# hruffieux/atlasqtl

Hardware: AMD Instinct MI355X
Metric: VB sweeps/sec (higher is better)
Workload: dtype f64; 1 GPU; atlasqtl VB sweep (S1-S22 incl. scheduled ELBO), n=1000 p=50000 q=10000, anneal=(1,2,10) on, horseshoe global-local, sweeps 6-93; n=1000, p=50000, q=10000, q_per_gpu=10000, parallelism=trait-sharded x1, env_overrides=

## Files before the change

atlasqtl_amd/csrc/aq_core_sweep_la.h:

```cpp
#pragma once
#include <hip/hip_runtime.h>
#include "aq_core_sweep.h"
#include <type_traits>

typedef double aq_v2 __attribute__((ext_vector_type(2)));

__device__ __forceinline__ double aq_row16_sum(double v) {
  auto step = [&](auto ctrl) __attribute__((always_inline)) {
    constexpr int C = decltype(ctrl)::value;
    const int lo = __builtin_amdgcn_update_dpp(0, __double2loint(v), C, 0xf, 0xf, false);
    const int hi = __builtin_amdgcn_update_dpp(0, __double2hiint(v), C, 0xf, 0xf, false);
    v += __hiloint2double(hi, lo);
  };
  step(std::integral_constant<int, 0xB1>{});
  step(std::integral_constant<int, 0x4E>{});
  step(std::integral_constant<int, 0x124>{});
  step(std::integral_constant<int, 0x128>{});
  return v;
}

#ifndef AQ_GLDS_AUX
#define AQ_GLDS_AUX 2
#endif
__device__ __forceinline__ void aq_glds16(const void *gsrc_lane, void *lds_base) {
  __builtin_amdgcn_global_load_lds((const __attribute__((address_space(1))) void *)gsrc_lane,
                                   (__attribute__((address_space(3))) void *)lds_base, 16, 0, AQ_GLDS_AUX);
}

template <int... Is, class F>
__device__ __forceinline__ void aq_static_for_impl(std::integer_sequence<int, Is...>, F &&f) {
  (f(std::integral_constant<int, Is>{}), ...);
}
template <int N, class F>
__device__ __forceinline__ void aq_static_for(F &&f) {
  aq_static_for_impl(std::make_integer_sequence<int, N>{}, f);
}

#define AQ_LD2(d0, d1, voff, sbase)                                                                            \
  do {                                                                                                          \
    const unsigned long long b_ = (unsigned long long)(sbase);                                                  \
    const unsigned lo_ = __builtin_amdgcn_readfirstlane((unsigned)b_);                                          \
    const unsigned hi_ = __builtin_amdgcn_readfirstlane((unsigned)(b_ >> 32));                                  \
    const unsigned long long u_ = ((unsigned long long)hi_ << 32) | lo_;                                        \
    asm volatile("global_load_dwordx4 %0, %2, %3\n\tglobal_load_dwordx4 %1, %2, %3 offset:1024"                \
                 : "=&v"(d0), "=&v"(d1)                                                                         \
                 : "v"(voff), "s"(u_));                                                                         \
  } while (0)
#define AQ_LD2I(d0, d1, voff, sbase, IMM)                                                                      \
  do {                                                                                                          \
    const unsigned long long b_ = (unsigned long long)(sbase);                                                  \
    const unsigned lo_ = __builtin_amdgcn_readfirstlane((unsigned)b_);                                          \
    const unsigned hi_ = __builtin_amdgcn_readfirstlane((unsigned)(b_ >> 32));                                  \
    const unsigned long long u_ = ((unsigned long long)hi_ << 32) | lo_;                                        \
    asm volatile("global_load_dwordx4 %0, %2, %3 offset:%4\n\tglobal_load_dwordx4 %1, %2, %3 offset:%5"        \
                 : "=&v"(d0), "=&v"(d1)                                                                         \
                 : "v"(voff), "s"(u_), "i"(IMM), "i"((IMM) + 1024));                                            \
  } while (0)
#define AQ_WAIT2(N, d0, d1) asm volatile("s_waitcnt vmcnt(" #N ")" : "+v"(d0), "+v"(d1))
template <int N>
__device__ __forceinline__ void aq_wait2n(aq_v2 &d0, aq_v2 &d1) {
  static_assert(N >= 0 && N < 64, "vmcnt is a 6-bit field");
  asm volatile("s_waitcnt vmcnt(%2)" : "+v"(d0), "+v"(d1) : "n"(N));
}

constexpr int aq_req_index(int D, int last, int stream , int k) {
  int n = 0;
  for (int j = 0; j <= D - 2; j++) {
    if (stream == 0 && k == j) return n;
    n++;
    if (j <= D - 3) {
      if (stream == 1 && k == j) return n;
      n++;
    }
  }
  for (int t = 0; t <= last; t++) {
    if (t + D - 1 <= last) {
      if (stream == 0 && k == t + D - 1) return n;
      n++;
    }
    if (t + D - 2 <= last) {
      if (stream == 1 && k == t + D - 2) return n;
      n++;
    }
  }
  return -1;
}
constexpr int aq_req_issued(int D, int last, int t) {
  int n = (D - 1) + (D - 2);
  for (int s = 0; s <= t; s++) n += (s + D - 1 <= last) + (s + D - 2 <= last);
  return n;
}
#ifndef AQ_DEEP_TT1
#define AQ_DEEP_TT1 4
#endif

template <int NT, int NT2, bool SEG, int TT, bool MASK = false, int NT3_ = -1, bool WIDE = false>
__global__ __launch_bounds__(8 * 64, 2) void aq_core_sweep_la_kernel(const AqCoreArgs a) {
  static_assert(!MASK || TT == 1, "the masked form keeps 16 per-trait Gram blocks in LDS: one trait tile per workgroup");
  static_assert(!WIDE || (TT == 1 && !SEG), "the wide sample split: one trait tile per workgroup, never chained");
  constexpr int NWM = 6;
  constexpr int NT3 = NT3_ >= 0 ? NT3_ : aq_la_nt3(NT, NT2, TT);
  constexpr int NPS = NWM + (NT3 > 0 ? 1 : 0);
  constexpr int NTR = 16 * TT;
  constexpr int ENT = 256 * TT;
  constexpr int NG = 4 / TT;
  constexpr int RPG = 16 / NG;
  const int tid = threadIdx.x;
  const int lane = tid & 63;
  const int w = tid >> 6;
  const bool is_rec = (w == 3);
  const int mw = w < 3 ? w : w - 1;
  const int g = lane >> 4;
  const int col = lane & 15;
  const int nwg = a.ntile / TT;
  int wg_ = blockIdx.x, seg_b0 = 0, seg_b1 = a.nb, seg = 0;
  if (SEG) {
    seg = blockIdx.x / nwg;
    wg_ = blockIdx.x - seg * nwg;
    seg_b0 = (int)((long long)a.nb * seg / a.nseg);
    seg_b1 = (int)((long long)a.nb * (seg + 1) / a.nseg);
    if (seg > 0) {
      if (tid == 0) {
        int tries = 0;
        while (__hip_atomic_load(&a.done[wg_], __ATOMIC_RELAXED, __HIP_MEMORY_SCOPE_AGENT) < seg) {
          __builtin_amdgcn_s_sleep(32);
          if (++tries > 4000000) { *a.errflag = 1; break; }
        }
        __builtin_amdgcn_fence(__ATOMIC_ACQUIRE, "agent");
        asm volatile("s_waitcnt vmcnt(0)" ::: "memory");
      }
      __syncthreads();
    }
  }
  const int C = SEG ? 1 : a.C;
  const int part = C > 1 ? wg_ % C : 0;
  const int wg = C > 1 ? wg_ / C : wg_;
  const bool lead = (part == 0);
  const int tile0 = wg * TT;
  const int nblk = seg_b1 - seg_b0;
  const bool helper = (w == 7);
  const int ht = lane & (NTR - 1), hg = lane / NTR;

  __shared__ double Sp[2][NPS][ENT];
  __shared__ double LA[2][ENT];
  __shared__ double Lm1[2][ENT];
  __shared__ double LB[2][ENT];
  __shared__ double Laa[2][ENT];
  __shared__ double LG[MASK ? 1 : 2][MASK ? 1 : 512];
  constexpr bool CXC = (TT == 1) && !MASK;
  __shared__ double LGx[MASK ? 1 : 3][MASK ? 1 : 256];
  __shared__ double LGk2[MASK ? 2 : 1][MASK ? AQ_GK_DIAG : 1];
  __shared__ double LGxk[MASK ? 4096 : 1];
  __shared__ double Lcoef[2][MASK ? ENT : 1], LK[2][MASK ? ENT : 1], Ls2[2][MASK ? ENT : 1], Lls2[2][MASK ? ENT : 1], Lxn[2][MASK ? ENT : 1];
  __shared__ double Lgam[2][ENT], Lmu[2][ENT], Ldel[2][ENT];
  __shared__ double Lcx[MASK ? 1 : ENT];
  __shared__ double Ldum[ENT];
  __shared__ double Stot[(SEG || TT == 2) ? 1 : 2][(SEG || TT == 2) ? 1 : ENT];
  __shared__ double Lpt[AQ_PT_LEN];
  __shared__ double Lred[6][64];
  __shared__ double Lrn[NPS * 4][NTR];
  __shared__ __attribute__((aligned(16))) int Fl[16];
  typedef __attribute__((address_space(3))) volatile int aq_lds_vint;
  aq_lds_vint *Flv = (aq_lds_vint *)(__attribute__((address_space(3))) int *)Fl;
  auto signal = [&](int idx, int val) __attribute__((always_inline)) {
    asm volatile("s_waitcnt lgkmcnt(0)" ::: "memory");
    if (lane == 0) Flv[idx] = val;
  };
#ifdef AQ_DIAG_TIME
  long long dg_wait = 0, dg_wait_b = 0;
  const long long dg_t0 = __builtin_readcyclecounter();
#endif
#if defined(AQ_DIAG_TIME) || defined(AQ_DIAG_TL)
  auto tl_mark = [&](int i, int k) __attribute__((always_inline)) {
    if (a.dbg && blockIdx.x == 0 && i >= 64 && i < 96 && lane == 0)
      a.dbg[(size_t)gridDim.x * 24 + ((size_t)w * 32 + (i - 64)) * 8 + k] = __builtin_readcyclecounter();
  };
#else
  auto tl_mark = [&](int, int) __attribute__((always_inline)) {};
#endif
  auto wait_ge = [&](int idx, int val) __attribute__((always_inline)) {
#ifdef AQ_DIAG_TIME
    const long long t_in = __builtin_readcyclecounter();
#endif
    while (Flv[idx] < val) __builtin_amdgcn_s_sleep(1);
    asm volatile("" ::: "memory");
#ifdef AQ_DIAG_TIME
    if (idx >= 7) dg_wait_b += __builtin_readcyclecounter() - t_in;
    else dg_wait += __builtin_readcyclecounter() - t_in;
#endif
  };
  typedef int aq_i4 __attribute__((ext_vector_type(4)));
  auto wait_s_and_staged = [&](int val) __attribute__((always_inline)) {
    typedef __attribute__((address_space(3))) volatile aq_i4 aq_lds_vi4;
    aq_lds_vi4 *fp = (aq_lds_vi4 *)(__attribute__((address_space(3))) int *)Fl;
#ifdef AQ_DIAG_TIME
    const long long t_in = __builtin_readcyclecounter();
#endif
    for (;;) {
      const aq_i4 f0 = fp[0], f1 = fp[1];
      const int lo = min(min(min(f0.x, f0.y), min(f0.z, f0.w)), min(min(f1.x, f1.y), f1.w));
      if (lo >= val) break;
      __builtin_amdgcn_s_sleep(1);
    }
    asm volatile("" ::: "memory");
#ifdef AQ_DIAG_TIME
    dg_wait += __builtin_readcyclecounter() - t_in;
#endif
  };
  if (tid < 16) Fl[tid] = 0;

  const int ktrait = tile0 * 16 + ht;
  const bool kvalid = ktrait < a.q;
  double sig2b_k = 1.0;
  if (helper) {
    sig2b_k = a.sig2b[ktrait];
    if (a.mode != 1)
      for (int e = lane; e < AQ_PT_LEN; e += 64) Lpt[e] = aq_pt_dev[e];
#pragma unroll
    for (int r = 0; r < RPG; r++) {
      const int e = lane + 64 * r;
      Ldel[0][e] = Ldel[1][e] = 0.0;
    }
    if constexpr (!MASK) {
#pragma unroll
      for (int r = 0; r < 4; r++) {
        const int e = lane + 64 * r;
        LG[0][(e >> 4) * 32 + 16 + (e & 15)] = 0.0;
        LG[1][(e >> 4) * 32 + 16 + (e & 15)] = 0.0;
      }
    }
  }

  constexpr int NTT = 3 * (NT + NT2) + NT3;
  const int nblk_s = a.mode == 1 ? 0 : nblk;
  auto run = [&](auto ntc, auto rolec, auto hook) __attribute__((always_inline)) {
    constexpr int NTC = decltype(ntc)::value;
    constexpr int ROLE = decltype(rolec)::value;
    constexpr bool HI = ROLE == 0;
    constexpr int ST = (NTC + 2) / 3;
    const int my_t0 = part * NTT + (ROLE == 0 ? mw * NT : ROLE == 1 ? 3 * NT + (mw - 3) * NT2 : 3 * (NT + NT2));
    const int slot = ROLE == 2 ? NWM : mw;
    aq_d4 Rr[TT][NTC];
    unsigned long long mb0 = 0, mb1 = 0;
    aq_static_for<TT>([&](auto ttc) __attribute__((always_inline)) {
      constexpr int tt = decltype(ttc)::value;
      const double *Rg = a.R + (size_t)(tile0 + tt) * a.n_pad * 16 + (size_t)(16 * my_t0 + g) * 16 + col;
      aq_static_for<NTC>([&](auto tc) __attribute__((always_inline)) {
        constexpr int t = decltype(tc)::value;
#pragma unroll
        for (int r = 0; r < 4; r++) Rr[tt][t][r] = Rg[(16 * t + 4 * r) * 16];
        if constexpr (MASK) {
          const double *Mg = a.mis + (size_t)tile0 * a.n_pad * 16 + (size_t)(16 * my_t0 + g) * 16 + col;
#pragma unroll
          for (int r = 0; r < 4; r++)
            if (Mg[(16 * t + 4 * r) * 16] != 0.0) { if (t < 16) mb0 |= 1ull << (4 * (t & 15) + r); else mb1 |= 1ull << (4 * (t & 15) + r); }
        }
      });
    });
    auto remask = [&](auto tc) __attribute__((always_inline)) {
      constexpr int t = decltype(tc)::value;
      const unsigned long long mb = t < 16 ? mb0 : mb1;
#pragma unroll
      for (int r = 0; r < 4; r++) Rr[0][t][r] = ((mb >> (4 * (t & 15) + r)) & 1ull) ? Rr[0][t][r] : 0.0;
    };
    const unsigned voff = (unsigned)((my_t0 * 128 + lane) * 16);
    const char *XUb = (const char *)a.XU, *XAb = (const char *)a.XA;
    const long long BLK = (long long)NTT * C * 128 * 16;
    aq_v2 p0, p1, q0, q1, c0, c1, d0, d1;
#ifdef AQ_FORCE_DEEP_DB
#ifdef AQ_FORCE_DEEP_TT2
    constexpr bool DEEP = (NTC >= 4);
#else
    constexpr bool DEEP = (TT == 1) && (NTC >= 4);
#endif
    constexpr int DB = !DEEP ? 1 : AQ_FORCE_DEEP_DB;
#elif defined(AQ_FORCE_DEEP_MASK_DB)
    constexpr bool DEEP = (TT == 1) && (NTC >= 4) && (MASK || true);
    constexpr int DB = !DEEP ? 1 : MASK ? AQ_FORCE_DEEP_MASK_DB : (NT <= 11) ? AQ_DEEP_TT1 : 3;
#else
    constexpr bool DEEP = (TT == 1) && (NTC >= 4) && (!MASK || (SEG && NT <= 11));
    constexpr int DB = !DEEP ? 1 : (!MASK && NT <= 11) ? AQ_DEEP_TT1 : 3;
#endif
    aq_v2 xb[DB][2], ab[DB][2];
    auto dangling = [&](const char *xu0, const char *xa0, auto skip_first) __attribute__((always_inline)) {
      aq_static_for<DB - 1>([&](auto jc) __attribute__((always_inline)) {
        constexpr int j = decltype(jc)::value;
        if constexpr (!(decltype(skip_first)::value && j == 0)) {
          constexpr int kb = (j + 2) / 4, imm = (j - 4 * kb) * 2048;
          AQ_LD2I(xb[j][0], xb[j][1], voff, xu0 + kb * 8192, imm);
        }
        if constexpr (j <= DB - 3) {
          constexpr int kb = (j + 2) / 4, imm = (j - 4 * kb) * 2048;
          AQ_LD2I(ab[j][0], ab[j][1], voff, xa0 + kb * 8192, imm);
        }
      });
    };
    if constexpr (DEEP) {
      dangling(XUb + seg_b0 * BLK, XAb + seg_b0 * BLK, std::false_type{});
    } else {
      AQ_LD2(p0, p1, voff, XUb + seg_b0 * BLK);
      AQ_LD2(c0, c1, voff, XAb + seg_b0 * BLK);
    }
    for (int i = 0; i <= nblk + 1; i++) {
      const bool do_u = i >= 2, do_s = i < nblk_s;
      const double mflag = do_u ? -1.0 : 0.0;
      const int bu = seg_b0 + (i >= 2 ? i - 2 : 0), bs = seg_b0 + (i < nblk ? i : nblk - 1);
      const int nbu = seg_b0 + (i >= 1 ? (i - 1 < nblk ? i - 1 : nblk - 1) : 0), nbs = seg_b0 + (i + 1 < nblk ? i + 1 : nblk - 1);
      tl_mark(i, 0);
      hook(i);
      tl_mark(i, 1);
      if (do_u && (ROLE != 2 || a.mode == 1)) wait_ge(6, i - 1);
      if (ROLE == 1 && a.stagger) wait_ge(8 + (mw - 3), i + 1);
      tl_mark(i, 2);
      double nd[TT][4];
      {
        unsigned zero = 0;
        asm volatile("" : "+v"(zero));
        const int ln = __builtin_amdgcn_mbcnt_hi(~0u, __builtin_amdgcn_mbcnt_lo(~0u, zero));
        const double *dl = &Ldel[bu & 1][(ln >> 4) * NTR + (ln & 15)];
#pragma unroll
        for (int tt = 0; tt < TT; tt++)
#pragma unroll
// ... 179 lines not shown
      __hip_atomic_store(&slot[(size_t)part * ENT + 64 * r], mine[r], __ATOMIC_RELAXED, __HIP_MEMORY_SCOPE_AGENT);
    }
    meanwhile();
    double tot[RPG];
#pragma unroll
    for (int r = 0; r < RPG; r++) tot[r] = 0.0;
    unsigned long long cur[RPG], nxt[RPG];
    auto request = [&](int c2, unsigned long long (&dst)[RPG]) __attribute__((always_inline)) {
#pragma unroll
      for (int r = 0; r < RPG; r++)
        dst[r] = __hip_atomic_load(&slot[(size_t)c2 * ENT + 64 * r], __ATOMIC_RELAXED, __HIP_MEMORY_SCOPE_AGENT);
    };
    request(part == 0 ? 1 : 0, cur);
    for (int c2 = 0; c2 < C; c2++) {
      if (c2 == part) {
#pragma unroll
        for (int r = 0; r < RPG; r++) tot[r] += __longlong_as_double((long long)mine[r]);
        continue;
      }
      int cn = c2 + 1;
      if (cn == part) cn++;
      if (cn < C) request(cn, nxt);
      int spins = 0;
      for (;;) {
        bool ok = true;
#pragma unroll
        for (int r = 0; r < RPG; r++) ok = ok && ((cur[r] & 3ull) == tag);
        if (__all(ok) || split_dead) break;
        __builtin_amdgcn_s_sleep(1);
        if (++spins > (1 << 22)) { *a.errflag = 1; split_dead = true; }
        request(c2, cur);
      }
#pragma unroll
      for (int r = 0; r < RPG; r++) {
        tot[r] += __longlong_as_double((long long)cur[r]);
        cur[r] = nxt[r];
      }
    }
#pragma unroll
    for (int r = 0; r < RPG; r++) own[r] = tot[r];
  };

  auto split_exchange_wide = [&](int b, double (&own)[RPG], auto meanwhile) __attribute__((always_inline)) {
    static_assert(RPG == 4 && ENT == 256, "one trait tile per workgroup");
    const int par = b & 1;
    const unsigned long long tag = 1ull + (unsigned long long)(((b - seg_b0) >> 1) % 3);
    unsigned long long *slots = (unsigned long long *)a.Pbuf + ((size_t)(wg * 2 + par) * (C + 1)) * ENT;
    tl_mark(b - seg_b0 + 1, 2);
#pragma unroll
    for (int r = 0; r < RPG; r++)
      __hip_atomic_store(&slots[(size_t)part * ENT + lane + 64 * r], ((unsigned long long)__double_as_longlong(own[r]) & ~3ull) | tag,
                         __ATOMIC_RELAXED, __HIP_MEMORY_SCOPE_AGENT);
    meanwhile();
    const int cmax = (ENT + C - 1) / C, nch = 64 / cmax, pc = (C + nch - 1) / nch;
    const int cnt = (ENT - 1 - part) / C + 1;
    const int i = lane / nch, k = lane - i * nch, c0 = k * pc;
    const bool act = i < cnt && c0 < C;
    const int e = part + C * i;
    unsigned long long v[AQ_LA_WPC];
    auto request = [&]() __attribute__((always_inline)) {
#pragma unroll
      for (int m = 0; m < AQ_LA_WPC; m++)
        if (act && m < pc && c0 + m < C)
          v[m] = __hip_atomic_load(&slots[(size_t)(c0 + m) * ENT + e], __ATOMIC_RELAXED, __HIP_MEMORY_SCOPE_AGENT);
    };
    request();
    for (int spins = 0;;) {
      bool ok = true;
#pragma unroll
      for (int m = 0; m < AQ_LA_WPC; m++)
        if (act && m < pc && c0 + m < C) ok = ok && ((v[m] & 3ull) == tag);
      if (__all(ok) || split_dead) break;
      __builtin_amdgcn_s_sleep(1);
      if (++spins > (1 << 22)) { *a.errflag = 1; split_dead = true; }
      request();
    }
    double acc = 0.0;
#pragma unroll
    for (int m = 0; m < AQ_LA_WPC; m++)
      if (act && m < pc && c0 + m < C) acc += __longlong_as_double((long long)v[m]);
    tl_mark(b - seg_b0 + 1, 3);
    double tot = acc;
    for (int kk = 1; kk < nch; kk++) {
      const double t = __shfl(acc, min(63, i * nch + kk), 64);
      if (kk * pc < C) tot += t;
    }
    if (act && k == 0)
      __hip_atomic_store(&slots[(size_t)C * ENT + e], ((unsigned long long)__double_as_longlong(tot) & ~3ull) | tag,
                         __ATOMIC_RELAXED, __HIP_MEMORY_SCOPE_AGENT);
    unsigned long long w4[RPG];
    auto request_tot = [&]() __attribute__((always_inline)) {
#pragma unroll
      for (int r = 0; r < RPG; r++) w4[r] = __hip_atomic_load(&slots[(size_t)C * ENT + lane + 64 * r], __ATOMIC_RELAXED, __HIP_MEMORY_SCOPE_AGENT);
    };
    request_tot();
    for (int spins = 0;;) {
      bool ok = true;
#pragma unroll
      for (int r = 0; r < RPG; r++) ok = ok && ((w4[r] & 3ull) == tag);
      if (__all(ok) || split_dead) break;
      __builtin_amdgcn_s_sleep(1);
      if (++spins > (1 << 22)) { *a.errflag = 1; split_dead = true; }
      request_tot();
    }
#pragma unroll
    for (int r = 0; r < RPG; r++) own[r] = __longlong_as_double((long long)w4[r]);
    tl_mark(b - seg_b0 + 1, 4);
  };

  __syncthreads();
  if (is_rec) {
    if (a.mode != 1) {
      const double rc_coef = MASK ? 0.0 : a.coef[ktrait];
      const double rc_cinv2s = MASK ? 0.0 : a.c * a.inv2s[ktrait];
      const double rc_K = rc_coef * rc_coef * rc_cinv2s;
      double cxn[CXC ? RPG : 1];
      auto chain_block = [&](int b) __attribute__((always_inline)) {
        const int par = b & 1;
        double Sown[RPG];
        const int need = b - seg_b0 + 1;
        if (C > 1 && a.xhelper) {
          wait_ge(14, need);
          wait_ge(7, need);
#pragma unroll
          for (int r = 0; r < RPG; r++) Sown[r] = Stot[par][(hg + NG * r) * NTR + ht];
        } else {
          wait_s_and_staged(need);
#pragma unroll
          for (int r = 0; r < RPG; r++) {
            const int j = hg + NG * r;
            double sv = Sp[par][0][j * NTR + ht];
#pragma unroll
            for (int ww = 1; ww < NPS; ww++) sv += Sp[par][ww][j * NTR + ht];
            Sown[r] = sv;
          }
        }
        tl_mark(need, 4);
        double cxs[(!SEG && TT == 1) ? RPG : 1];
        auto correction = [&](auto subc) __attribute__((always_inline)) {
          constexpr bool sub = decltype(subc)::value;
          if constexpr (CXC) {
#pragma unroll
            for (int r = 0; r < RPG; r++) {
              const double cx = b > seg_b0 ? cxn[r] : 0.0;
              if constexpr (sub) Sown[r] -= cx;
              else cxs[r] = cx;
            }
          } else if constexpr (!MASK) {
            if (b > seg_b0) {
              wait_ge(12, need);
#pragma unroll
              for (int r = 0; r < RPG; r++) {
                const double cx = Lcx[lane + 64 * r];
                if constexpr (sub) Sown[r] -= cx;
                else cxs[r] = cx;
              }
            } else if constexpr (!sub) {
#pragma unroll
              for (int r = 0; r < RPG; r++) cxs[r] = 0.0;
            }
          } else if (b > seg_b0) {
            double dlp[16];
#pragma unroll
            for (int i = 0; i < 16; i++) dlp[i] = Ldel[par ^ 1][i * NTR + ht];
#pragma unroll
            for (int r = 0; r < RPG; r++) {
              double cx = 0.0;
              const double *gx = &LGxk[((hg + NG * r) * 16) * 16 + ht];
#pragma unroll
              for (int i = 0; i < 16; i++) cx += gx[i * 16] * dlp[i];
              if constexpr (sub) Sown[r] -= cx;
              else cxs[r] = cx;
            }
          } else if constexpr (!sub) {
#pragma unroll
            for (int r = 0; r < RPG; r++) cxs[r] = 0.0;
          }
        };
        bool corrected = false;
        if constexpr (!SEG && TT == 1) {
          if (C > 1 && !a.xhelper) {
            if constexpr (WIDE) split_exchange_wide(b, Sown, [&]() __attribute__((always_inline)) { correction(std::false_type{}); });
            else split_exchange(b, Sown, [&]() __attribute__((always_inline)) { correction(std::false_type{}); });
#pragma unroll
            for (int r = 0; r < RPG; r++) Sown[r] -= cxs[r];
            corrected = true;
          }
        }
        if (!corrected) correction(std::true_type{});
        tl_mark(need, 5);
        double sb = __shfl(Sown[0], ht, 64);
        double s_nx = __shfl(Sown[1 / NG], (1 % NG) * NTR + ht, 64);
        typedef __attribute__((address_space(3))) double aq_lds_double;
        const bool wsel = lane < NTR;
        aq_lds_double *wdum = (aq_lds_double *)Ldum + ht;
        aq_lds_double *wgam = wsel ? (aq_lds_double *)Lgam[par] + ht : wdum;
        aq_lds_double *wmu = wsel ? (aq_lds_double *)Lmu[par] + ht : wdum;
        aq_lds_double *wdel = wsel ? (aq_lds_double *)Ldel[par] + ht : wdum;
        if constexpr (MASK) {
          signal(13, b - seg_b0 + 1);
          const double *LGk = &LGk2[par][0];
          int rtri[RPG], rrow[RPG];
#pragma unroll
          for (int r = 0; r < RPG; r++) { rrow[r] = hg + NG * r; rtri[r] = rrow[r] * (rrow[r] + 1) / 2; }
          double m1o = Lm1[par][ht], cA = LA[par][ht], cf = Lcoef[par][ht], ci = LK[par][ht], dj = LGk[ht];
#pragma unroll
          for (int j = 0; j < 16; j++) {
            const int jn = (j + 1) & 15, j2 = j + 2;
            const int en = jn * NTR + ht;
            double m1o_n = Lm1[par][en], cA_n = LA[par][en], cf_n = Lcoef[par][en], ci_n = LK[par][en];
            double d_n = LGk[(jn * (jn + 1) / 2 + jn) * 16 + ht];
            const double g_next = LGk[(j < 15 ? (jn * (jn + 1) / 2 + j) : 0) * 16 + ht];
            const int r2 = (j2 & 15) / NG;
            double gl[RPG];
#pragma unroll
            for (int r = (j / NG); r < RPG; r++) gl[r] = LGk[(rtri[r] + (rrow[r] < j ? rrow[r] : j)) * 16 + ht];
            __builtin_amdgcn_sched_barrier(0);
            double s = sb + m1o * dj;
            double mu = cf * s;
            double x = fma(-(s * s), ci, cA);
            double gm = aq_sigmoid_neg_fast(x);
            double dl = gm * mu - m1o;
            sb = s_nx - g_next * dl;
            auto upd = [&](int r) __attribute__((always_inline)) { Sown[r] -= gl[r] * dl; };
            if (j2 < 16) {
              Sown[r2] -= gl[r2] * dl;
              s_nx = __shfl(Sown[r2], (j2 % NG) * NTR + ht, 64);
              __builtin_amdgcn_sched_barrier(0);
            }
#pragma unroll
            for (int r = (j / NG); r < RPG; r++)
              if (!(j2 < 16 && r == j2 / NG)) upd(r);
            wgam[j * NTR] = gm;
            wmu[j * NTR] = mu;
            wdel[j * NTR] = dl;
            m1o = m1o_n; cA = cA_n; cf = cf_n; ci = ci_n; dj = d_n;
          }
        } else {
        double m1o = Lm1[par][ht], cA = LA[par][ht], dj = LG[par][0];
#pragma unroll
        for (int j = 0; j < 16; j++) {
          const int jn = (j + 1) & 15, j2 = j + 2;
          double m1o_n = Lm1[par][jn * NTR + ht], cA_n = LA[par][jn * NTR + ht], d_n = LG[par][jn * 33];
          const double g_next = LG[par][j * 32 + jn];
          double gl[RPG];
#pragma unroll
          for (int r = (j / NG); r < RPG; r++) gl[r] = LG[par][j * 32 + hg + NG * r];
          double gxn[CXC ? RPG : 1];
          if constexpr (CXC) {
#pragma unroll
            for (int r = 0; r < RPG; r++) gxn[r] = LGx[(b + 1) % 3][(hg + NG * r) * 16 + j];
          }
          __builtin_amdgcn_sched_barrier(0);
          double s = sb + m1o * dj;
          double mu = rc_coef * s;
          double x = fma(-(s * s), rc_K, cA);
          double gm = aq_sigmoid_neg_fast(x);
          double dl = gm * mu - m1o;
          sb = s_nx - g_next * dl;
          if (j2 < 16) {
            Sown[j2 / NG] -= gl[j2 / NG] * dl;
            s_nx = __shfl(Sown[j2 / NG], (j2 % NG) * NTR + ht, 64);
            __builtin_amdgcn_sched_barrier(0);
          }
#pragma unroll
          for (int r = (j / NG); r < RPG; r++)
            if (!(j2 < 16 && r == j2 / NG)) Sown[r] -= gl[r] * dl;
          if constexpr (CXC) {
#pragma unroll
            for (int r = 0; r < RPG; r++) cxn[r] = (j == 0 ? 0.0 : cxn[r]) + gxn[r] * dl;
          }
          wgam[j * NTR] = gm;
          wmu[j * NTR] = mu;
          wdel[j * NTR] = dl;
          m1o = m1o_n; cA = cA_n; dj = d_n;
          if (j == 7) tl_mark(need, 6);
        }
        }
        signal(6, b - seg_b0 + 1);
      };
      if constexpr (NT3 > 0) {
        run(std::integral_constant<int, (NT3 > 0 ? NT3 : 1)>{}, std::integral_constant<int, 2>{},
            [&](int i) __attribute__((always_inline)) { if (i >= 1 && i <= nblk) chain_block(seg_b0 + i - 1); });
      } else {
        for (int b = seg_b0; b < seg_b1; b++) chain_block(b);
      }
    } else if constexpr (NT3 > 0) {
      run(std::integral_constant<int, (NT3 > 0 ? NT3 : 1)>{}, std::integral_constant<int, 2>{}, no_hook);
    }
    __syncthreads();
  } else if (helper) {
    if (a.hprio == 3) __builtin_amdgcn_s_setprio(3);
    else if (a.hprio == 2) __builtin_amdgcn_s_setprio(2);
    else if (a.hprio == 1) __builtin_amdgcn_s_setprio(1);
    const size_t tbase = (size_t)(tile0 + (ht >> 4)) * a.p_pad * 16 + (ht & 15);
    const double zk = a.zeta[ktrait];
    typedef __attribute__((address_space(3))) const double aq_lds_cdouble;
    aq_lds_cdouble *ptab = (aq_lds_cdouble *)(__attribute__((address_space(3))) double *)Lpt;
    const double inv_sqrt_c = 1.0 / a.sqrt_c;
    const double cst_k = MASK ? 0.0 : a.cst[ktrait];
    double th[RPG];
    auto theta_load = [&](int b) __attribute__((always_inline)) {
#pragma unroll
      for (int r = 0; r < RPG; r++) th[r] = a.theta[16 * b + hg + NG * r];
    };
    double pg[MASK ? 1 : RPG], pm[MASK ? 1 : RPG];
    auto gm_load = [&](int b) __attribute__((always_inline)) {
      if constexpr (!MASK) {
#pragma unroll
        for (int r = 0; r < RPG; r++) {
          const size_t off = tbase + (size_t)(16 * b + hg + NG * r) * 16;
          pg[r] = a.gam[off];
          pm[r] = a.mu[off];
        }
      }
    };
    const double tau_k = MASK ? a.tau[ktrait] : 1.0;
    const double sig2_inv_h = MASK ? *a.sig2_inv_p : 0.0;
    const double cstna_k = MASK ? -(a.log_tau[ktrait] + *a.log_sig2_inv_p) / 2 : 0.0;
    auto gk_block = [&](int b) __attribute__((always_inline)) { return a.GK + ((size_t)tile0 * a.nb + b) * AQ_GK_STRIDE; };
    auto gk_dma = [&](int b, int par) __attribute__((always_inline)) {
      const char *src = (const char *)gk_block(b) + lane * 16;
#pragma unroll
      for (int i = 0; i < AQ_GK_DIAG / 128; i++) aq_glds16(src + 1024 * i, &LGk2[par][128 * i]);
      src += AQ_GK_DIAG * 8;
#pragma unroll
      for (int i = 0; i < 32; i++) aq_glds16(src + 1024 * i, &LGxk[128 * i]);
    };
    double pl_g[MASK ? RPG : 1], pl_m[MASK ? RPG : 1], pl_xn[MASK ? RPG : 1];
    double sv_g[MASK ? RPG : 1], sv_m[MASK ? RPG : 1], sv_xn[MASK ? RPG : 1], sv_th[MASK ? RPG : 1];
    auto pre_load = [&](int b) __attribute__((always_inline)) {
      const double *gk = gk_block(b);
#pragma unroll
      for (int r = 0; r < RPG; r++) {
        const size_t off = tbase + (size_t)(16 * b + hg + NG * r) * 16;
        const int jj = hg + NG * r;
        pl_g[r] = a.gam[off];
        pl_m[r] = a.mu[off];
        pl_xn[r] = gk[(jj * (jj + 1) / 2 + jj) * 16 + ht];
      }
    };
    auto stage_dma = [&](int b, int par, int b_next) __attribute__((always_inline)) {
#pragma unroll
      for (int r = 0; r < RPG; r++) {
        asm volatile("" : "+v"(pl_g[r]), "+v"(pl_m[r]), "+v"(pl_xn[r]), "+v"(th[r]) : : "memory");
        sv_g[r] = pl_g[r]; sv_m[r] = pl_m[r]; sv_xn[r] = pl_xn[r]; sv_th[r] = th[r];
      }
      gk_dma(b, par);
      if (b_next < seg_b1) { pre_load(b_next); theta_load(b_next); }
    };
    auto stage = [&](int b, int par) __attribute__((always_inline)) {
      double st_G[4], st_Gx[4], st_xn[MASK ? RPG : 1];
      if constexpr (MASK) {
#pragma unroll
        for (int r = 0; r < RPG; r++) { Lm1[par][lane + 64 * r] = sv_g[r] * sv_m[r]; st_xn[r] = sv_xn[r]; }
      } else {
#pragma unroll
        for (int r = 0; r < RPG; r++) Lm1[par][lane + 64 * r] = pg[r] * pm[r];
#pragma unroll
        for (int r = 0; r < 4; r++) {
          st_G[r] = a.G[(size_t)b * 256 + lane + 64 * r];
          const int bx = CXC ? (b + 1 < a.nb ? b + 1 : b) : b;
          st_Gx[r] = a.Gx[(size_t)bx * 256 + lane + 64 * r];
        }
      }
      double ls2r[MASK ? RPG : 1];
      if constexpr (MASK) {
#pragma unroll
        for (int r = 0; r < RPG; r++) {
          const int e = lane + 64 * r;
          const double is2 = a.c * (st_xn[r] + sig2_inv_h) * tau_k;
          const double s2 = aq_recip_pos(is2);
          const double ls2 = -aq_log_pos(is2);
          const double cf = a.c * s2 * tau_k;
          Lcoef[par][e] = cf;
          LK[par][e] = cf * cf * (a.c * 0.5 * is2);
          Ls2[par][e] = s2;
          Lls2[par][e] = ls2;
          Lxn[par][e] = st_xn[r];
          ls2r[r] = ls2;
        }
      }
      auto emitA = [&](int r, double A) __attribute__((always_inline)) {
        const int j = 16 * b + hg + NG * r, e = lane + 64 * r;
        const bool valid = kvalid && j < a.p;
        if constexpr (MASK) {
          LA[par][e] = a.c * ((valid ? A : 0.0) - 0.5 * ls2r[r] + cstna_k);
        } else {
          LA[par][e] = a.c * ((valid ? A : 0.0) + cst_k);
        }
      };
      auto emitZ = [&](int r, double zb, double za) __attribute__((always_inline)) {
        const int j = 16 * b + hg + NG * r, e = lane + 64 * r;
        const bool valid = kvalid && j < a.p;
        LB[par][e] = valid ? zb : 0.0;
        Laa[par][e] = valid ? za : 0.0;
      };
      auto emit2 = [&](int r, double A, double zb, double za) __attribute__((always_inline)) {
        const int j = 16 * b + hg + NG * r, e = lane + 64 * r;
        const bool valid = kvalid && j < a.p;
        LB[par][e] = valid ? zb : 0.0;
        Laa[par][e] = valid ? za : 0.0;
        if constexpr (MASK) LA[par][e] = a.c * ((valid ? A : 0.0) - 0.5 * Lls2[par][e] + cstna_k);
        else LA[par][e] = a.c * ((valid ? A : 0.0) + cst_k);
      };
      double uu[RPG];
      bool inr = true;
#pragma unroll
      for (int r = 0; r < RPG; r++) {
        uu[r] = (MASK ? sv_th[r] : th[r]) + zk;
        inr = inr && fabs(uu[r]) < AQ_PT_R && fabs(a.sqrt_c * uu[r]) < AQ_PT_R;
      }
      {
        constexpr int NC = AQ_PT_DEG + 1, S = AQ_PT_NI, F = NC * S;
        auto locate = [&](double x, double *xloc) __attribute__((always_inline)) {
          const double t = fmin(fabs(x) * (1.0 / AQ_PT_W), AQ_PT_NI - 0.5);
          const int i = (int)t;
          *xloc = fma(2.0, t - (double)i, -1.0);
          return ptab + i;
        };
        {
          double co[2][NC], xl[2];
          auto fetch = [&](int r, auto setc) __attribute__((always_inline)) {
            constexpr int set = decltype(setc)::value;
            aq_lds_cdouble *pp = locate(uu[r], &xl[set]);
#pragma unroll
            for (int k = 0; k < NC; k++) co[set][k] = pp[k * S];
          };
          fetch(0, std::integral_constant<int, 0>{});
          aq_static_for<RPG>([&](auto rc) __attribute__((always_inline)) {
            constexpr int r = decltype(rc)::value, set = r & 1;
            if constexpr (r + 1 < RPG) fetch(r + 1, std::integral_constant<int, (r + 1) & 1>{});
            __builtin_amdgcn_sched_barrier(0);
            double pa = co[set][NC - 1];
#pragma unroll
            for (int k = NC - 2; k >= 0; k--) pa = fma(pa, xl[set], co[set][k]);
            emitA(r, uu[r] < 0.0 ? -pa : pa);
            __builtin_amdgcn_sched_barrier(0);
          });
        }
        {
          double co[2][2 * NC], xl[2];
          auto fetch = [&](int r, auto setc) __attribute__((always_inline)) {
            constexpr int set = decltype(setc)::value;
            aq_lds_cdouble *pp = locate(a.sqrt_c * uu[r], &xl[set]);
#pragma unroll
            for (int k = 0; k < NC; k++) {
              co[set][k] = pp[F + k * S];
              co[set][NC + k] = pp[2 * F + k * S];
            }
          };
          fetch(0, std::integral_constant<int, 0>{});
          aq_static_for<RPG>([&](auto rc) __attribute__((always_inline)) {
            constexpr int r = decltype(rc)::value, set = r & 1;
            if constexpr (r + 1 < RPG) fetch(r + 1, std::integral_constant<int, (r + 1) & 1>{});
            __builtin_amdgcn_sched_barrier(0);
            double pb = co[set][NC - 1], pd = co[set][2 * NC - 1];
#pragma unroll
            for (int k = NC - 2; k >= 0; k--) {
              pb = fma(pb, xl[set], co[set][k]);
              pd = fma(pd, xl[set], co[set][NC + k]);
            }
            const double d = uu[r] < 0.0 ? -pd : pd;
            emitZ(r, pb * inv_sqrt_c, uu[r] - 0.5 * inv_sqrt_c * (pb + d));
            __builtin_amdgcn_sched_barrier(0);
          });
        }
      }
      if (__builtin_expect(!__all(inr), 0)) {
#pragma unroll 1
        for (int r = 0; r < RPG; r++) {
          double ur = uu[0];
#pragma unroll
          for (int k = 1; k < RPG; k++) ur = (r == k) ? uu[k] : ur;
          double A, bM, dM, dummy;
          aq_probit_tab_eval<1>(ur, ptab, &A, &dummy, &dummy);
          aq_probit_tab_eval<2>(a.sqrt_c * ur, ptab, &dummy, &bM, &dM);
          emit2(r, A, bM * inv_sqrt_c, ur - 0.5 * inv_sqrt_c * (bM + dM));
        }
      }
      if constexpr (MASK) {
#ifdef AQ_DIAG_TIME
        const long long t_dma = __builtin_readcyclecounter();
#endif
        asm volatile("s_waitcnt vmcnt(0)" ::: "memory");
#ifdef AQ_DIAG_TIME
        dg_wait += __builtin_readcyclecounter() - t_dma;
#endif
      } else {
#pragma unroll
        for (int r = 0; r < 4; r++) {
          const int e = lane + 64 * r;
          LG[par][(e >> 4) * 32 + (e & 15)] = st_G[r];
          LGx[CXC ? (b + 1) % 3 : par][e] = st_Gx[r];
        }
      }
    };
    double cs0 = 0.0, cs1 = 0.0, cs2 = 0.0, cs3 = 0.0, cs5 = 0.0;
    auto finalize = [&](int b, int par) __attribute__((always_inline)) {
#pragma unroll
      for (int r = 0; r < RPG; r++) {
        const int e = lane + 64 * r, hj = hg + NG * r;
        const double gm = Lgam[par][e], mu = Lmu[par][e];
        const size_t off = tbase + (size_t)(16 * b + hj) * 16;
        if (lead) {
          a.gam[off] = gm;
          a.mu[off] = mu;
        }
        const int j = 16 * b + hj;
        double gb = 0.0;
        if (kvalid && j < a.p) {
          const double be = gm * mu;
          gb = Laa[par][e] + gm * LB[par][e];
          cs0 += gm;
          cs3 += gb;
          if constexpr (MASK) {
            const double s2 = Ls2[par][e];
            const double m2 = (mu * mu + s2) * gm;
            const double xn = Lxn[par][e];
            cs1 += m2;
            cs2 += xn * (m2 - be * be);
            cs5 += gm * Lls2[par][e];
          } else {
            cs1 += (mu * mu + sig2b_k) * gm;
            cs2 += be * be;
          }
        }
        gb = aq_row16_sum(gb);
        if ((ht & 15) == 0 && lead) a.rowGB[(size_t)(tile0 + (ht >> 4)) * a.p_pad + j] = gb;
      }
    };
    auto exchange = [&](int b) __attribute__((always_inline)) {
      const int par = b & 1, kdone = b - seg_b0 + 1;
      if constexpr (WIDE) tl_mark(kdone, 0);
#pragma unroll
      for (int m = 0; m < NWM; m++) wait_ge(m, kdone);
      if constexpr (NT3 > 0) wait_ge(11, kdone);
      if constexpr (WIDE) tl_mark(kdone, 1);
      double own[RPG];
#pragma unroll
      for (int r = 0; r < RPG; r++) {
        const int e = lane + 64 * r;
        double sv = Sp[par][0][e];
#pragma unroll
        for (int ww = 1; ww < NPS; ww++) sv += Sp[par][ww][e];
        own[r] = sv;
      }
      if constexpr (WIDE) split_exchange_wide(b, own, [] {});
      else split_exchange(b, own, [] {});
#pragma unroll
      for (int r = 0; r < RPG; r++) Stot[par][lane + 64 * r] = own[r];
      signal(14, kdone);
    };
    if (a.mode == 1) {
      for (int b = seg_b0; b < seg_b1; b++) {
        const int k = b - seg_b0, par = b & 1;
        if (k >= 2) {
#pragma unroll
          for (int m = 0; m < NWM; m++) wait_ge(m, k + 1);
          if (NT3 > 0) wait_ge(11, k + 1);
        }
#pragma unroll
        for (int r = 0; r < RPG; r++) {
          const int e = lane + 64 * r, hj = hg + NG * r;
          const size_t off = tbase + (size_t)(16 * b + hj) * 16;
          double gm = a.gam[off], mu = a.mu[off];
          double be = gm * mu;
          Ldel[par][e] = be;
          if (kvalid && (16 * b + hj) < a.p) {
            const double m2 = (mu * mu + sig2b_k) * gm;
            cs0 += gm;
            cs1 += m2;
            if constexpr (MASK) cs2 += gk_block(b)[(hj * (hj + 1) / 2 + hj) * 16 + ht] * (m2 - be * be);
            else cs2 += be * be;
          }
        }
        signal(6, k + 1);
      }
    } else {
      int xt[8] = {0, 0, 0, 0, 0, 0, 0, 0};
      const long long xt_blk = (long long)NTT * C * 2048;
      const int xt_nsl = (int)((xt_blk + 8191) / 8192);
      const int xt_wg = (int)(gridDim.x < 256 ? gridDim.x : 256) / 8 > 0 ? (int)(gridDim.x < 256 ? gridDim.x : 256) / 8 : 1;
      auto x_touch = [&](int bA, int bU) __attribute__((always_inline)) {
        asm volatile("s_waitcnt vmcnt(0)" : "+v"(xt[0]), "+v"(xt[1]), "+v"(xt[2]), "+v"(xt[3]), "+v"(xt[4]), "+v"(xt[5]), "+v"(xt[6]), "+v"(xt[7]));
        const char *pa = (const char *)a.XA + (long long)bA * xt_blk + lane * 128, *pu = (const char *)a.XU + (long long)bU * xt_blk + lane * 128;
#pragma unroll
        for (int k = 0; k < 4; k++) {
          const int sl = (int)((blockIdx.x >> 3) % xt_wg) + k * xt_wg;
          if (sl < xt_nsl && (long long)sl * 8192 + lane * 128 < xt_blk) {
            asm volatile("global_load_dword %0, %1, off" : "=v"(xt[2 * k]) : "v"(pa + (long long)sl * 8192));
            asm volatile("global_load_dword %0, %1, off" : "=v"(xt[2 * k + 1]) : "v"(pu + (long long)sl * 8192));
          }
        }
      };
      theta_load(seg_b0);
      gm_load(seg_b0);
      if constexpr (MASK) { pre_load(seg_b0); stage_dma(seg_b0, seg_b0 & 1, seg_b0 + 1); }
      stage(seg_b0, seg_b0 & 1);
      signal(7, 1);
      if constexpr (!SEG && TT == 1) { if (C > 1 && a.xhelper) exchange(seg_b0); }
      if constexpr (!MASK) { if (seg_b0 + 1 < seg_b1) { theta_load(seg_b0 + 1); gm_load(seg_b0 + 1); } }
      for (int b = seg_b0; b < seg_b1; b++) {
        const int par = b & 1;
        if constexpr (MASK) {
          if (b + 1 < seg_b1) { wait_ge(13, b - seg_b0 + 1); stage_dma(b + 1, par ^ 1, b + 2); }
        }
        if (b > seg_b0) {
          wait_ge(6, b - seg_b0);
          if constexpr (!MASK && !CXC) {
            double dlp[16];
#pragma unroll
            for (int i = 0; i < 16; i++) dlp[i] = Ldel[par ^ 1][i * NTR + ht];
#pragma unroll
            for (int r = 0; r < RPG; r++) {
              double cx = 0.0;
              const double *gx = &LGx[par][(hg + NG * r) * 16];
#pragma unroll
              for (int i = 0; i < 16; i++) cx += gx[i] * dlp[i];
              Lcx[lane + 64 * r] = cx;
            }
            signal(12, b - seg_b0 + 1);
          }
          finalize(b - 1, par ^ 1);
        }
        if (b + 1 < seg_b1) {
          stage(b + 1, par ^ 1);
          signal(7, b - seg_b0 + 2);
          if constexpr (!SEG && TT == 1) { if (C > 1 && a.xhelper) exchange(b + 1); }
          if (a.xtouch && b + 2 < seg_b1) x_touch(b + 2, b);
          if constexpr (!MASK) { if (b + 2 < seg_b1) { theta_load(b + 2); gm_load(b + 2); } }
        }
      }
      asm volatile("s_waitcnt vmcnt(0)" : "+v"(xt[0]), "+v"(xt[1]), "+v"(xt[2]), "+v"(xt[3]), "+v"(xt[4]), "+v"(xt[5]), "+v"(xt[6]), "+v"(xt[7]));
      wait_ge(6, nblk);
      finalize(seg_b1 - 1, (seg_b1 - 1) & 1);
    }
    Lred[0][lane] = cs0; Lred[1][lane] = cs1; Lred[2][lane] = cs2; Lred[3][lane] = cs3; Lred[5][lane] = cs5;
    __syncthreads();
  } else {
    if (mw < 3) run(std::integral_constant<int, NT>{}, std::integral_constant<int, 0>{}, no_hook);
    else run(std::integral_constant<int, NT2>{}, std::integral_constant<int, 1>{}, no_hook);
    __syncthreads();
  }
#ifdef AQ_DIAG_TIME
  if (lane == 0 && a.dbg) {
    a.dbg[((size_t)blockIdx.x * 8 + w) * 3] = dg_wait;
    a.dbg[((size_t)blockIdx.x * 8 + w) * 3 + 1] = dg_wait_b;
    a.dbg[((size_t)blockIdx.x * 8 + w) * 3 + 2] = __builtin_readcyclecounter() - dg_t0;
  }
#endif
  if (tid < NTR) {
    int k2 = tile0 * 16 + tid;
    double r2 = 0.0;
    for (int s = 0; s < NPS * 4; s++) r2 += Lrn[s][tid];
    double *sm = a.sums + (size_t)seg * (MASK ? 6 : 5) * a.q_pad;
    if (C > 1) a.rnpart[(size_t)part * a.q_pad + k2] = r2;
    else sm[(size_t)4 * a.q_pad + k2] = r2;
    for (int v = 0; v < 6 && lead; v++) {
      if (v == 4 || (v == 5 && !MASK)) continue;
      double acc2 = 0.0;
      for (int jj = 0; jj < NG; jj++) acc2 += Lred[v][jj * NTR + tid];
      sm[(size_t)v * a.q_pad + k2] = acc2;
    }
  }
  if (SEG) {
    asm volatile("s_waitcnt vmcnt(0)" ::: "memory");
    __syncthreads();
    if (tid == 0) {
      __builtin_amdgcn_fence(__ATOMIC_RELEASE, "agent");
      asm volatile("s_waitcnt vmcnt(0)" ::: "memory");
      __hip_atomic_store(&a.done[wg], seg + 1, __ATOMIC_RELAXED, __HIP_MEMORY_SCOPE_AGENT);
    }
  }
}
```

Before: 29.39 sweeps/s.

## Specialize helper stage/finalize for full blocks and c=1, batch row16 reductions

Splits the helper wave's per-block stage into head/tab/tail parts and adds compile-time specializations for blocks fully inside p and q (skipping validity checks) and for c==1, where the second probit table lookup reuses the first and the scaling by inv_sqrt_c is dropped. Replaces the per-element 16-lane DPP reductions in finalize with a batched transpose-and-reduce that sums RPG values using lane selects plus two DPP steps, so that four lanes each write several row sums. Also simplifies address arithmetic for the gamma/mu loads and stores and uses scalar-base global loads in the prefetch-touch path. Adds code size and register pressure from the extra template instantiations, and the batched reduction depends on the lane ownership mapping being correct.

Result: no change. 29.44 sweeps/s, median of 6 (+0.2%).

```diff
diff --git a/atlasqtl_amd/csrc/aq_core_sweep_la.h b/atlasqtl_amd/csrc/aq_core_sweep_la.h
--- a/atlasqtl_amd/csrc/aq_core_sweep_la.h
+++ b/atlasqtl_amd/csrc/aq_core_sweep_la.h
@@ -5,19 +5,59 @@
 
 typedef double aq_v2 __attribute__((ext_vector_type(2)));
 
+template <int CTRL>
+__device__ __forceinline__ double aq_dpp_f64(double v) {
+  const int lo = __builtin_amdgcn_mov_dpp(__double2loint(v), CTRL, 0xf, 0xf, false);
+  const int hi = __builtin_amdgcn_mov_dpp(__double2hiint(v), CTRL, 0xf, 0xf, false);
+  return __hiloint2double(hi, lo);
+}
 __device__ __forceinline__ double aq_row16_sum(double v) {
-  auto step = [&](auto ctrl) __attribute__((always_inline)) {
-    constexpr int C = decltype(ctrl)::value;
-    const int lo = __builtin_amdgcn_update_dpp(0, __double2loint(v), C, 0xf, 0xf, false);
-    const int hi = __builtin_amdgcn_update_dpp(0, __double2hiint(v), C, 0xf, 0xf, false);
-    v += __hiloint2double(hi, lo);
-  };
-  step(std::integral_constant<int, 0xB1>{});
-  step(std::integral_constant<int, 0x4E>{});
-  step(std::integral_constant<int, 0x124>{});
-  step(std::integral_constant<int, 0x128>{});
+  v += aq_dpp_f64<0xB1>(v);
+  v += aq_dpp_f64<0x4E>(v);
+  v += aq_dpp_f64<0x124>(v);
+  v += aq_dpp_f64<0x128>(v);
   return v;
 }
+__device__ __forceinline__ double aq_lane_select(double a, double b, unsigned long long mask) {
+  int lo, hi;
+  asm("v_cndmask_b32_e64 %0, %1, %2, %3" : "=v"(lo) : "v"(__double2loint(a)), "v"(__double2loint(b)), "s"(mask));
+  asm("v_cndmask_b32_e64 %0, %1, %2, %3" : "=v"(hi) : "v"(__double2hiint(a)), "v"(__double2hiint(b)), "s"(mask));
+  return __hiloint2double(hi, lo);
+}
+template <bool XOR1>
+__device__ __forceinline__ double aq_lane_select_swap(double a, double b, unsigned long long mask) {
+  int lo, hi;
+  if constexpr (XOR1)
+    asm("v_cndmask_b32_e64 %0, %2, %4, %6\n\tv_cndmask_b32_e64 %1, %3, %5, %6\n\ts_nop 0\n\t"
+        "v_mov_b32_dpp %0, %0 quad_perm:[1,0,3,2] row_mask:0xf bank_mask:0xf\n\t"
+        "v_mov_b32_dpp %1, %1 quad_perm:[1,0,3,2] row_mask:0xf bank_mask:0xf"
+        : "=&v"(lo), "=&v"(hi)
+        : "v"(__double2loint(a)), "v"(__double2hiint(a)), "v"(__double2loint(b)), "v"(__double2hiint(b)), "s"(mask));
+  else
+    asm("v_cndmask_b32_e64 %0, %2, %4, %6\n\tv_cndmask_b32_e64 %1, %3, %5, %6\n\ts_nop 0\n\t"
+        "v_mov_b32_dpp %0, %0 quad_perm:[2,3,0,1] row_mask:0xf bank_mask:0xf\n\t"
+        "v_mov_b32_dpp %1, %1 quad_perm:[2,3,0,1] row_mask:0xf bank_mask:0xf"
+        : "=&v"(lo), "=&v"(hi)
+        : "v"(__double2loint(a)), "v"(__double2hiint(a)), "v"(__double2loint(b)), "v"(__double2hiint(b)), "s"(mask));
+  return __hiloint2double(hi, lo);
+}
+template <int N>
+__device__ __forceinline__ void aq_row16_sum(double (&v)[N]) {
+  static_assert(N % 4 == 0, "two halving steps");
+  constexpr unsigned long long ODD = 0xAAAAAAAAAAAAAAAAull, HI2 = 0xCCCCCCCCCCCCCCCCull;
+#pragma unroll
+  for (int i = 0; i < N / 2; i++)
+    v[i] = aq_lane_select(v[i], v[i + N / 2], ODD) + aq_lane_select_swap<true>(v[i + N / 2], v[i], ODD);
+#pragma unroll
+  for (int i = 0; i < N / 4; i++)
+    v[i] = aq_lane_select(v[i], v[i + N / 4], HI2) + aq_lane_select_swap<false>(v[i + N / 4], v[i], HI2);
+#pragma unroll
+  for (int i = 0; i < N / 4; i++) v[i] += aq_dpp_f64<0x124>(v[i]);
+#pragma unroll
+  for (int i = 0; i < N / 4; i++) v[i] += aq_dpp_f64<0x128>(v[i]);
+}
+template <int N>
+__device__ __forceinline__ int aq_row16_owner(int lane, int i) { return i + (N / 4) * ((lane >> 1) & 1) + (N / 2) * (lane & 1); }
 
 #ifndef AQ_GLDS_AUX
 #define AQ_GLDS_AUX 2
@@ -803,16 +843,17 @@
     double th[RPG];
     auto theta_load = [&](int b) __attribute__((always_inline)) {
 #pragma unroll
-      for (int r = 0; r < RPG; r++) th[r] = a.theta[16 * b + hg + NG * r];
+      for (int r = 0; r < RPG; r++) th[r] = (a.theta + (16 * b + hg))[NG * r];
     };
     double pg[MASK ? 1 : RPG], pm[MASK ? 1 : RPG];
     auto gm_load = [&](int b) __attribute__((always_inline)) {
       if constexpr (!MASK) {
+        const size_t off0 = tbase + (size_t)(16 * b + hg) * 16;
+        const double *const gp = a.gam + off0, *const mp = a.mu + off0;
 #pragma unroll
         for (int r = 0; r < RPG; r++) {
-          const size_t off = tbase + (size_t)(16 * b + hg + NG * r) * 16;
-          pg[r] = a.gam[off];
-          pm[r] = a.mu[off];
+          pg[r] = gp[r * (NG * 16)];
+          pm[r] = mp[r * (NG * 16)];
         }
       }
     };
@@ -850,8 +891,9 @@
       gk_dma(b, par);
       if (b_next < seg_b1) { pre_load(b_next); theta_load(b_next); }
     };
-    auto stage = [&](int b, int par) __attribute__((always_inline)) {
-      double st_G[4], st_Gx[4], st_xn[MASK ? RPG : 1];
+    double st_G[4], st_Gx[4], ls2r[MASK ? RPG : 1];
+    auto stage_head = [&](int b, int par) __attribute__((always_inline)) {
+      double st_xn[MASK ? RPG : 1];
       if constexpr (MASK) {
 #pragma unroll
         for (int r = 0; r < RPG; r++) { Lm1[par][lane + 64 * r] = sv_g[r] * sv_m[r]; st_xn[r] = sv_xn[r]; }
@@ -865,7 +907,6 @@
           st_Gx[r] = a.Gx[(size_t)bx * 256 + lane + 64 * r];
         }
       }
-      double ls2r[MASK ? RPG : 1];
       if constexpr (MASK) {
 #pragma unroll
         for (int r = 0; r < RPG; r++) {
@@ -882,9 +923,12 @@
           ls2r[r] = ls2;
         }
       }
+    };
+    auto stage_tab = [&](int b, int par, auto fullc, auto c1c) __attribute__((always_inline)) {
+      constexpr bool FULL = decltype(fullc)::value, C1 = decltype(c1c)::value;
       auto emitA = [&](int r, double A) __attribute__((always_inline)) {
         const int j = 16 * b + hg + NG * r, e = lane + 64 * r;
-        const bool valid = kvalid && j < a.p;
+        const bool valid = FULL || (kvalid && j < a.p);
         if constexpr (MASK) {
           LA[par][e] = a.c * ((valid ? A : 0.0) - 0.5 * ls2r[r] + cstna_k);
         } else {
@@ -893,24 +937,16 @@
       };
       auto emitZ = [&](int r, double zb, double za) __attribute__((always_inline)) {
         const int j = 16 * b + hg + NG * r, e = lane + 64 * r;
-        const bool valid = kvalid && j < a.p;
+        const bool valid = FULL || (kvalid && j < a.p);
         LB[par][e] = valid ? zb : 0.0;
         Laa[par][e] = valid ? za : 0.0;
       };
-      auto emit2 = [&](int r, double A, double zb, double za) __attribute__((always_inline)) {
-        const int j = 16 * b + hg + NG * r, e = lane + 64 * r;
-        const bool valid = kvalid && j < a.p;
-        LB[par][e] = valid ? zb : 0.0;
-        Laa[par][e] = valid ? za : 0.0;
-        if constexpr (MASK) LA[par][e] = a.c * ((valid ? A : 0.0) - 0.5 * Lls2[par][e] + cstna_k);
-        else LA[par][e] = a.c * ((valid ? A : 0.0) + cst_k);
-      };
       double uu[RPG];
       bool inr = true;
 #pragma unroll
       for (int r = 0; r < RPG; r++) {
         uu[r] = (MASK ? sv_th[r] : th[r]) + zk;
-        inr = inr && fabs(uu[r]) < AQ_PT_R && fabs(a.sqrt_c * uu[r]) < AQ_PT_R;
+        inr = inr && fabs(uu[r]) < AQ_PT_R && (C1 || fabs(a.sqrt_c * uu[r]) < AQ_PT_R);
       }
       {
         constexpr int NC = AQ_PT_DEG + 1, S = AQ_PT_NI, F = NC * S;
@@ -920,11 +956,14 @@
           *xloc = fma(2.0, t - (double)i, -1.0);
           return ptab + i;
         };
+        aq_lds_cdouble *pk[C1 ? RPG : 1];
+        double xk[C1 ? RPG : 1];
         {
           double co[2][NC], xl[2];
           auto fetch = [&](int r, auto setc) __attribute__((always_inline)) {
             constexpr int set = decltype(setc)::value;
             aq_lds_cdouble *pp = locate(uu[r], &xl[set]);
+            if constexpr (C1) { pk[r] = pp; xk[r] = xl[set]; }
 #pragma unroll
             for (int k = 0; k < NC; k++) co[set][k] = pp[k * S];
           };
@@ -944,7 +983,9 @@
           double co[2][2 * NC], xl[2];
           auto fetch = [&](int r, auto setc) __attribute__((always_inline)) {
             constexpr int set = decltype(setc)::value;
-            aq_lds_cdouble *pp = locate(a.sqrt_c * uu[r], &xl[set]);
+            aq_lds_cdouble *pp;
+            if constexpr (C1) { pp = pk[r]; xl[set] = xk[r]; }
+            else pp = locate(a.sqrt_c * uu[r], &xl[set]);
 #pragma unroll
             for (int k = 0; k < NC; k++) {
               co[set][k] = pp[F + k * S];
@@ -963,17 +1004,27 @@
               pd = fma(pd, xl[set], co[set][NC + k]);
             }
             const double d = uu[r] < 0.0 ? -pd : pd;
-            emitZ(r, pb * inv_sqrt_c, uu[r] - 0.5 * inv_sqrt_c * (pb + d));
+            if constexpr (C1) emitZ(r, pb, uu[r] - 0.5 * (pb + d));
+            else emitZ(r, pb * inv_sqrt_c, uu[r] - 0.5 * inv_sqrt_c * (pb + d));
             __builtin_amdgcn_sched_barrier(0);
           });
         }
       }
+      return inr;
+    };
+    auto stage_tail = [&](int b, int par, bool inr) __attribute__((always_inline)) {
+      auto emit2 = [&](int r, double A, double zb, double za) __attribute__((always_inline)) {
+        const int j = 16 * b + hg + NG * r, e = lane + 64 * r;
+        const bool valid = kvalid && j < a.p;
+        LB[par][e] = valid ? zb : 0.0;
+        Laa[par][e] = valid ? za : 0.0;
+        if constexpr (MASK) LA[par][e] = a.c * ((valid ? A : 0.0) - 0.5 * Lls2[par][e] + cstna_k);
+        else LA[par][e] = a.c * ((valid ? A : 0.0) + cst_k);
+      };
       if (__builtin_expect(!__all(inr), 0)) {
 #pragma unroll 1
         for (int r = 0; r < RPG; r++) {
-          double ur = uu[0];
-#pragma unroll
-          for (int k = 1; k < RPG; k++) ur = (r == k) ? uu[k] : ur;
+          const double ur = a.theta[16 * b + hg + NG * r] + zk;
           double A, bM, dM, dummy;
           aq_probit_tab_eval<1>(ur, ptab, &A, &dummy, &dummy);
           aq_probit_tab_eval<2>(a.sqrt_c * ur, ptab, &dummy, &bM, &dM);
@@ -998,23 +1049,39 @@
       }
     };
     double cs0 = 0.0, cs1 = 0.0, cs2 = 0.0, cs3 = 0.0, cs5 = 0.0;
-    auto finalize = [&](int b, int par) __attribute__((always_inline)) {
+    const bool kall = tile0 * 16 + NTR <= a.q;
+    auto whole = [&](int b) __attribute__((always_inline)) { return kall && 16 * b + 16 <= a.p; };
+    const bool c_is_1 = a.sqrt_c == 1.0;
+    auto stage_block = [&](int b, int par) __attribute__((always_inline)) {
+      stage_head(b, par);
+      bool inr;
+      if (!MASK && whole(b)) {
+        if (c_is_1) inr = stage_tab(b, par, std::true_type{}, std::true_type{});
+        else inr = stage_tab(b, par, std::true_type{}, std::false_type{});
+      } else {
+        inr = stage_tab(b, par, std::false_type{}, std::false_type{});
+      }
+      stage_tail(b, par, inr);
+    };
+    auto finalize = [&](int b, int par, auto fullc) __attribute__((always_inline)) {
+      constexpr bool FULL = decltype(fullc)::value;
+      const size_t off0 = tbase + (size_t)(16 * b + hg) * 16;
+      double *const gp = a.gam + off0, *const mp = a.mu + off0;
+      double gb[RPG];
 #pragma unroll
       for (int r = 0; r < RPG; r++) {
-        const int e = lane + 64 * r, hj = hg + NG * r;
+        const int e = lane + 64 * r;
         const double gm = Lgam[par][e], mu = Lmu[par][e];
-        const size_t off = tbase + (size_t)(16 * b + hj) * 16;
         if (lead) {
-          a.gam[off] = gm;
-          a.mu[off] = mu;
-        }
-        const int j = 16 * b + hj;
-        double gb = 0.0;
-        if (kvalid && j < a.p) {
+          gp[r * (NG * 16)] = gm;
+          mp[r * (NG * 16)] = mu;
+        }
+        gb[r] = 0.0;
+        if (FULL || (kvalid && 16 * b + hg + NG * r < a.p)) {
           const double be = gm * mu;
-          gb = Laa[par][e] + gm * LB[par][e];
+          gb[r] = Laa[par][e] + gm * LB[par][e];
           cs0 += gm;
-          cs3 += gb;
+          cs3 += gb[r];
           if constexpr (MASK) {
             const double s2 = Ls2[par][e];
             const double m2 = (mu * mu + s2) * gm;
@@ -1027,9 +1094,17 @@
             cs2 += be * be;
           }
         }
-        gb = aq_row16_sum(gb);
-        if ((ht & 15) == 0 && lead) a.rowGB[(size_t)(tile0 + (ht >> 4)) * a.p_pad + j] = gb;
-      }
+      }
+      aq_row16_sum(gb);
+      if ((ht & 15) < 4 && lead) {
+        double *const rp = a.rowGB + (size_t)(tile0 + (ht >> 4)) * a.p_pad + (16 * b + hg) + aq_row16_owner<RPG>(lane, 0) * NG;
+#pragma unroll
+        for (int i = 0; i < RPG / 4; i++) rp[i * NG] = gb[i];
+      }
+    };
+    auto finalize_block = [&](int b, int par) __attribute__((always_inline)) {
+      if (whole(b)) finalize(b, par, std::true_type{});
+      else finalize(b, par, std::false_type{});
     };
     auto exchange = [&](int b) __attribute__((always_inline)) {
       const int par = b & 1, kdone = b - seg_b0 + 1;
@@ -1085,20 +1160,21 @@
       const int xt_wg = (int)(gridDim.x < 256 ? gridDim.x : 256) / 8 > 0 ? (int)(gridDim.x < 256 ? gridDim.x : 256) / 8 : 1;
       auto x_touch = [&](int bA, int bU) __attribute__((always_inline)) {
         asm volatile("s_waitcnt vmcnt(0)" : "+v"(xt[0]), "+v"(xt[1]), "+v"(xt[2]), "+v"(xt[3]), "+v"(xt[4]), "+v"(xt[5]), "+v"(xt[6]), "+v"(xt[7]));
-        const char *pa = (const char *)a.XA + (long long)bA * xt_blk + lane * 128, *pu = (const char *)a.XU + (long long)bU * xt_blk + lane * 128;
+        const char *pa = (const char *)a.XA + (long long)bA * xt_blk, *pu = (const char *)a.XU + (long long)bU * xt_blk;
 #pragma unroll
         for (int k = 0; k < 4; k++) {
           const int sl = (int)((blockIdx.x >> 3) % xt_wg) + k * xt_wg;
           if (sl < xt_nsl && (long long)sl * 8192 + lane * 128 < xt_blk) {
-            asm volatile("global_load_dword %0, %1, off" : "=v"(xt[2 * k]) : "v"(pa + (long long)sl * 8192));
-            asm volatile("global_load_dword %0, %1, off" : "=v"(xt[2 * k + 1]) : "v"(pu + (long long)sl * 8192));
+            asm volatile("global_load_dword %0, %1, %2" : "=v"(xt[2 * k]) : "v"(lane * 128), "s"(pa + (long long)sl * 8192));
+            asm volatile("global_load_dword %0, %1, %2" : "=v"(xt[2 * k + 1]) : "v"(lane * 128), "s"(pu + (long long)sl * 8192));
           }
         }
       };
       theta_load(seg_b0);
       gm_load(seg_b0);
       if constexpr (MASK) { pre_load(seg_b0); stage_dma(seg_b0, seg_b0 & 1, seg_b0 + 1); }
-      stage(seg_b0, seg_b0 & 1);
+      stage_head(seg_b0, seg_b0 & 1);
+      stage_tail(seg_b0, seg_b0 & 1, stage_tab(seg_b0, seg_b0 & 1, std::false_type{}, std::false_type{}));
       signal(7, 1);
       if constexpr (!SEG && TT == 1) { if (C > 1 && a.xhelper) exchange(seg_b0); }
       if constexpr (!MASK) { if (seg_b0 + 1 < seg_b1) { theta_load(seg_b0 + 1); gm_load(seg_b0 + 1); } }
@@ -1123,10 +1199,10 @@
             }
             signal(12, b - seg_b0 + 1);
           }
-          finalize(b - 1, par ^ 1);
+          finalize_block(b - 1, par ^ 1);
         }
         if (b + 1 < seg_b1) {
-          stage(b + 1, par ^ 1);
+          stage_block(b + 1, par ^ 1);
           signal(7, b - seg_b0 + 2);
           if constexpr (!SEG && TT == 1) { if (C > 1 && a.xhelper) exchange(b + 1); }
           if (a.xtouch && b + 2 < seg_b1) x_touch(b + 2, b);
@@ -1135,7 +1211,7 @@
       }
       asm volatile("s_waitcnt vmcnt(0)" : "+v"(xt[0]), "+v"(xt[1]), "+v"(xt[2]), "+v"(xt[3]), "+v"(xt[4]), "+v"(xt[5]), "+v"(xt[6]), "+v"(xt[7]));
       wait_ge(6, nblk);
-      finalize(seg_b1 - 1, (seg_b1 - 1) & 1);
+      finalize(seg_b1 - 1, (seg_b1 - 1) & 1, std::false_type{});
     }
     Lred[0][lane] = cs0; Lred[1][lane] = cs1; Lred[2][lane] = cs2; Lred[3][lane] = cs3; Lred[5][lane] = cs5;
     __syncthreads();
```
